# ASSERT-KTH/QuantizedSAE

Measured on AMD Instinct MI355X. Metric: activations/sec, BinarySAE 512->32768 n_bits=4 forward (dense latent + reconstruction + MSE), higher is better.
Workload: dtype f32; 1 GPU; BinarySAE(512, 32768, gamma=4.0, n_bits=4) k=65, 65536 rows per GPU per step, reference forward() signature (dense [B,32768] latent, [B,512] reconstruction, polarize loss) + recon-MSE accumulation; rows_per_gpu=65536, input_dim=512, hidden_dim=32768, n_bits=4, top_k=65, parallelism=row-sharded x1, no data-path collective, batches_in_flight=2

## Files before the change

quantizedsae_amd/_lib.py:

```python
from __future__ import annotations

import ctypes as C
from pathlib import Path
from typing import Optional

_PKG = Path(__file__).resolve().parent
import os

LIB_PATH = Path(os.environ["QSAE_HIP_LIB"]) if os.environ.get("QSAE_HIP_LIB") else _PKG / "lib" / "libqsae_hip.so"
DEBUG_LIB_PATH = _PKG / "lib" / "libqsae_hip_debug.so"
ABI_VERSION = 4

OK = 0
ERR_INVALID_ARG, ERR_UNSUPPORTED, ERR_HIP, ERR_WORKSPACE = -1, -2, -3, -4
ACT_NONE, ACT_RELU, ACT_SIGMOID = 0, 1, 2

_vp, _i, _i64, _f, _sz = C.c_void_p, C.c_int, C.c_int64, C.c_float, C.c_size_t

SIGNATURES = {
    "qsae_abi_version": (_i, []),
    "qsae_last_error": (C.c_char_p, []),
    "qsae_device_info": (_i, [C.POINTER(_i), C.c_char_p, _i]),
    "qsae_profile_sweep_events": (_i, [_vp, _vp]),
    "qsae_profile_event_create": (_i, [C.POINTER(_vp)]),
# ... 222 lines not shown
    "qsaej_threshold_grad": (_i, [_vp, _vp, _vp, _vp, _vp, _i, _i, _i, _f, _vp, _vp]),
}

JUMP_DENSE_SIGNATURES = {
    "qsaed_encode_jump_workspace_bytes": (_sz, [_i, _i, _i, _i]),
    "qsaed_encode_jump": (_i, [_vp, _i64, _vp, _i64, _vp, _vp, _i, _i, _i, _i, _f, _f, _vp, _vp, _vp, _vp, _vp, _vp, _vp, _vp, _sz,
                               _vp]),
}

BATCH_DENSE_SIGNATURES = {
    "qsaebd_encode_batch_topk_workspace_bytes": (_sz, [_i, _i, _i, _i]),
    "qsaebd_encode_batch_topk": (_i, [_vp, _i64, _vp, _i64, _vp, _i, _i, _i, _i, _i64, _vp, _f, _f, _vp, _vp, _vp, _vp, _vp, _vp,
                                      _f, _vp, _sz, _vp]),
}


class QsaeError(RuntimeError):

    def __init__(self, code: int, message: str):
        super().__init__(f"libqsae_hip error {code}: {message}")
        self.code = code


_libs = {}
_active = "product"


def _open(path: Path) -> C.CDLL:
    if not path.exists():
        raise RuntimeError(
            f"{path} is missing: build it with `python -m quantizedsae_amd.build` "
            "(hipcc --offload-arch=gfx950).  quantizedsae_amd has no CPU / eager fallback.")
    lib = C.CDLL(str(path))
    for name, (res, args) in list(SIGNATURES.items()) + list(EXT_SIGNATURES.items()) + list(CURVE_SIGNATURES.items()) \
            + list(NESTED_SIGNATURES.items()) + list(BATCH_SIGNATURES.items()) + list(NESTED_BATCH_SIGNATURES.items()) + list(MULTIK_SIGNATURES.items()) \
            + list(JUMP_SIGNATURES.items()) + list(JUMP_DENSE_SIGNATURES.items()) \
            + list(BATCH_DENSE_SIGNATURES.items()):
        fn = getattr(lib, name)
        fn.restype = res
        fn.argtypes = args
    if lib.qsae_abi_version() != ABI_VERSION:
        raise RuntimeError(f"{path.name}: ABI version mismatch; rebuild it")
    return lib


def load() -> C.CDLL:
    lib = _libs.get(_active)
    if lib is None:
        lib = _libs[_active] = _open(LIB_PATH if _active == "product" else DEBUG_LIB_PATH)
    return lib


# ... 23 lines not shown
```

quantizedsae_amd/build.py:

```python
from __future__ import annotations

import os
import shutil
import subprocess
from concurrent.futures import ThreadPoolExecutor
from pathlib import Path

PKG = Path(__file__).resolve().parent
CSRC = PKG / "csrc"
LIBDIR = PKG / "lib"
LIB = LIBDIR / "libqsae_hip.so"
DEBUG_LIB = LIBDIR / "libqsae_hip_debug.so"
OBJDIR = PKG / "lib" / "obj"

SOURCES = ["encode.hip", "topk.hip", "binary.hip", "dense_dec.hip", "encode_topk.hip", "prefilter_topk.hip", "encode_bits.hip",
           "encode_emu.hip", "misc.hip", "analysis.hip", "coactivation_bits.hip", "coactivation_partners.hip", "token_overlap.hip", "token_lists.hip", "dictionary.hip", "dictionary_neighbors.hip", "dictionary_neighbors_f32.hip", "kmeans.hip", "top_examples.hip", "evaluation.hip", "train.hip", "train_gemm.hip",
           "train_mask.hip", "optim.hip", "trainer.hip", "watch.hip", "activity.hip", "resample.hip", "auxk.hip",
           "sparsity_curve.hip", "nested.hip", "batch_topk.hip", "batch_topk_decode.hip", "nested_ragged.hip", "multi_topk.hip", "jumprelu.hip",
           "jump_dense.hip", "batch_dense.hip"]
HEADERS = sorted(p.name for p in (Path(__file__).resolve().parent / "csrc").glob("*.h"))
ARCH = "gfx950"
FLAGS = ["-O3", f"--offload-arch={ARCH}", "-ffp-contract=off", "-fPIC", "-std=c++17", "-Wall",
         "-Wno-unused-function", "-Wno-unused-variable"]

# ... 7 lines not shown

def _stale(target: Path, deps) -> bool:
    if not target.exists():
        return True
    t = target.stat().st_mtime
    return any(Path(d).stat().st_mtime > t for d in deps)


def build_native(force: bool = False, verbose: bool = False, debug: bool = False) -> Path:
    srcs = [CSRC / s for s in SOURCES if (CSRC / s).exists()]
    hdrs = [CSRC / h for h in HEADERS] + [PKG.parent / "include" / "qsae.h", PKG.parent / "include" / "qsae_ext.h",
                                        PKG.parent / "include" / "qsae_curve.h", PKG.parent / "include" / "qsae_nested.h",
                                        PKG.parent / "include" / "qsae_batch.h", PKG.parent / "include" / "qsae_nested_batch.h",
                                        PKG.parent / "include" / "qsae_multik.h", PKG.parent / "include" / "qsae_jump.h",
                                        PKG.parent / "include" / "qsae_jump_dense.h",
                                        PKG.parent / "include" / "qsae_batch_dense.h"]
    objdir = OBJDIR / "debug" if debug else OBJDIR
    lib = DEBUG_LIB if debug else LIB
    flags = FLAGS + (["-DQSAE_DEBUG_BUILD=1"] if debug else [])
    objdir.mkdir(parents=True, exist_ok=True)
    hipcc = _hipcc()
    jobs = []
    for src in srcs:
        obj = objdir / (src.stem + ".o")
        if force or _stale(obj, [src] + hdrs):
            jobs.append((src, obj))

    def compile_one(job):
        src, obj = job
        cmd = [hipcc] + flags + ["-c", str(src), "-o", str(obj)]
        if verbose:
# ... 30 lines not shown
```

quantizedsae_amd/csrc/encode_topk_internal.h:

```cpp
#pragma once

#include "gemm_mfma_f32_dma.h"
#include "decode_row.h"

namespace qsae {

int topk_rows_dispatch(float* latent, int64_t ld, int B, int H, int k, int32_t* idx, float* val, int zero_rest,
                       float* tau, uint2* cand, int* cnt, int cap, float* dense, int64_t dense_ld, hipStream_t s,
                       const float* margin = nullptr, int stride = 0);
int scatter_rows(const int32_t* idx, const float* val, int B, int k, int H, float* dense, int64_t ld, hipStream_t s);
int decode_binary_sparse_rows(const int* rows, int nrows, const int32_t* idx, const float* val, int k, int H,
                              const RowDecode& d, hipStream_t s);
int densify_rows(const int32_t* idx, const float* val, int B, int k, int H, float* dense, int64_t ld, hipStream_t s);
int gather_rows(const float* src, const int* rows, int n, int D, float* dst, hipStream_t s);
void launch_x_prep(const float* x, int B, int D, const float* meta, _Float16* xq, float* inv, float* margin, hipStream_t s,
                   int* zero_word = nullptr);

constexpr int kChunkRows = 1024;
constexpr int kTopkMaxH = 32768;
constexpr int kCandCap = 1024;
constexpr int kMaxSpecRows = kChunkRows;
constexpr int kRefMaxD = 2048;
constexpr int kRefTileStride = 36;

#ifdef QSAE_DEBUG_BUILD
// ... 157 lines not shown
```

quantizedsae_amd/csrc/misc.hip:

```cpp
#include <map>

#include "common.h"

namespace qsae {

char* last_error_buf() {
    static thread_local char buf[512] = {0};
    return buf;
}

int thread_device_ctx(ThreadDeviceCtx** out) {
    static thread_local std::map<int, ThreadDeviceCtx> table;
    int dev = -1;
    QSAE_HIP(hipGetDevice(&dev));
    auto it = table.find(dev);
    if (it == table.end()) {
        ThreadDeviceCtx c{};
        auto undo = [&c]() {
            if (c.pinned) (void)hipHostFree(c.pinned);
            if (c.ev_copied) (void)hipEventDestroy(c.ev_copied);
            if (c.ev_join) (void)hipEventDestroy(c.ev_join);
            if (c.ev_fork) (void)hipEventDestroy(c.ev_fork);
            if (c.side) (void)hipStreamDestroy(c.side);
        };
// ... 22 lines not shown
}

typedef float f32x4 __attribute__((ext_vector_type(4)));

__global__ void __launch_bounds__(256)
scatter_rows_kernel(const int32_t* __restrict__ idx, const float* __restrict__ val, long long total, int k,
                    int H, float* __restrict__ dense, int64_t ld) {
    const long long gid = static_cast<long long>(blockIdx.x) * blockDim.x + threadIdx.x;
    if (gid >= total) return;
    const long long b = gid / k;
    const int h = idx[gid];
    if (h >= 0 && h < H) dense[b * ld + h] = val[gid];
}

__global__ void __launch_bounds__(256)
sq_err_kernel(const float* __restrict__ r, const float* __restrict__ x, size_t n, double* __restrict__ sum) {
    const size_t n4 = n / 4;
    double acc = 0.0;
    const size_t stride = static_cast<size_t>(gridDim.x) * blockDim.x;
    const size_t tiles = n4 / 1024;
    double acc1 = 0.0;
    for (size_t t = blockIdx.x; t < tiles; t += gridDim.x) {
        const size_t i0 = t * 1024 + threadIdx.x;
        f32x4 a[4], b[4];
#pragma unroll
        for (int u = 0; u < 4; ++u) {
            a[u] = reinterpret_cast<const f32x4*>(r)[i0 + 256 * u];
            b[u] = reinterpret_cast<const f32x4*>(x)[i0 + 256 * u];
        }
#pragma unroll
// ... 95 lines not shown
        QSAE_HIP(hipMemset2DAsync(dense, static_cast<size_t>(ld) * sizeof(float), 0,
                                  static_cast<size_t>(H) * sizeof(float), B, s));
    }
    return scatter_rows(idx, val, B, k, H, dense, ld, s);
}

int scatter_rows(const int32_t* idx, const float* val, int B, int k, int H, float* dense, int64_t ld, hipStream_t s) {
    const long long total = static_cast<long long>(B) * k;
    if (total == 0) return QSAE_OK;
    hipLaunchKernelGGL(scatter_rows_kernel, dim3(static_cast<unsigned>((total + 255) / 256)), dim3(256), 0, s, idx,
                       val, total, k, H, dense, ld);
    QSAE_LAUNCH_CHECK();
    return QSAE_OK;
}

}

using namespace qsae;

extern "C" int qsae_kperm_rows(const float* src, int rows, int K, float* dst, qsae_stream_t stream) {
    QSAE_CHECK_ARG(rows >= 0 && K > 0, "rows >= 0 and K > 0 required");
    if (rows == 0) return QSAE_OK;
    QSAE_CHECK_ARG(src && dst && src != dst, "null or aliasing pointers");
    QSAE_CHECK_SUPPORTED(K % 8 == 0, "K must be a multiple of 8");
    QSAE_CHECK_ARG(aligned16(src) && aligned16(dst), "src and dst must be 16-byte aligned");
    const long long groups = static_cast<long long>(rows) * (K / 8);
    hipLaunchKernelGGL(kperm_rows_kernel, dim3(static_cast<unsigned>((groups + 255) / 256)), dim3(256), 0,
                       as_stream(stream), src, groups, dst);
    QSAE_LAUNCH_CHECK();
    return QSAE_OK;
// ... 129 lines not shown
```

quantizedsae_amd/csrc/prefilter_topk.hip:

```cpp
#ifdef QSAE_DEBUG_BUILD
#define QSAE_DEFINE_SHARED_TUNABLES 1
#endif
#include "encode_topk_internal.h"
#include "sweep_xstat_f16.h"
#include "refine_row.h"
#include "refine_sliced.h"

namespace qsae {

constexpr int kFillCoWaves = 1024;
constexpr int kFillCoPace = 3;

QSAE_TUNABLE_PTR g_xstat_stamps = nullptr;
QSAE_TUNABLE g_fuse_xprep = 0;
QSAE_TUNABLE g_inkernel_pilot = 1;
QSAE_TUNABLE g_inkernel_rank = 0;
QSAE_TUNABLE g_pilot_tile = 0;
QSAE_TUNABLE g_fill_in_sweep = 1;
QSAE_TUNABLE g_fill_co = 1;
QSAE_TUNABLE g_xstat_ablate = 0;
QSAE_TUNABLE g_x_parts = 0;
QSAE_TUNABLE g_pref_tile = 2;

struct PrefLayout {
// ... 228 lines not shown
    return fits == 1;
}

static int launch_fill_co(ThreadDeviceCtx* ctx, float* dense, int64_t dense_ld, int B, int H, hipStream_t s) {
    QSAE_HIP(hipStreamWaitEvent(ctx->side, ctx->ev_fork, 0));
    hipLaunchKernelGGL(co_delay_kernel, dim3(1), dim3(64), 0, ctx->side, 2000);
    QSAE_LAUNCH_CHECK();
    hipLaunchKernelGGL(fill_zero_co_kernel, dim3(g_fill_co > 1 ? g_fill_co % 10000 : kFillCoWaves), dim3(64), 0, ctx->side,
                       dense, static_cast<long long>(dense_ld), B, H / 256, g_fill_co > 1 ? g_fill_co / 10000 : kFillCoPace);
    QSAE_LAUNCH_CHECK();
    QSAE_HIP(hipEventRecord(ctx->ev_join, ctx->side));
    QSAE_HIP(hipStreamWaitEvent(s, ctx->ev_join, 0));
    return QSAE_OK;
}

static bool prefilter_shape_ok(int B, int D, int H, int k) {
    return use_fused(B, D, H, k) && D % 64 == 0 && D <= kRefMaxD && (H - pilot_width(H)) > 0;
}

static int inkernel_rank(int k) {
    const double target = 5.0 * k > 200.0 ? 5.0 * k : 200.0;
    int r = static_cast<int>(32.0 * (1.0 - exp(-target / 512.0)) + 0.5);
    return r < 6 ? 6 : (r > 24 ? 24 : r);
}

struct PrefCall {
    const float* x; const float* W; const float* bias; const _Float16* Wq; const float* meta;
    int B, D, H, k;
    int32_t* idx; float* val;
    char* ws; qsae_stream_t stream;
    float* dense; int64_t dense_ld;
    const RowDecode* dec;
};
struct PrefPlan {
    FusedLayout L; PrefLayout PL;
    int P;
    bool xstat, inkernel, fill_co, fill_in_sweep;
    int Hs, hoff, parts, cap_part;
    float* filled;
};
static PrefPlan pref_plan(const PrefCall& c) {
    PrefPlan p;
    p.L = fused_layout(c.B, c.D, c.H, c.k);
    p.PL = pref_layout(c.B, c.D, p.L.total);
    p.P = pilot_width(c.H);
    p.xstat = g_pref_tile == 2 && xstat_supported(c.D, c.H - p.P, p.P) && c.H % 4 == 0;
    p.inkernel = p.xstat && g_inkernel_pilot && p.P % kXsHT == 0 && c.H % kXsHT == 0 && xstat_supported(c.D, c.H, 0);
    p.Hs = p.inkernel ? c.H : c.H - p.P;
    p.hoff = p.inkernel ? 0 : p.P;
    p.parts = p.xstat ? (g_x_parts > 0 ? g_x_parts : xstat_parts(c.B, p.Hs, kCandCap)) : 1;
    p.cap_part = kCandCap / p.parts;
    p.fill_co = p.xstat && c.dense && g_fill_co && c.D == 512 && c.H % 256 == 0 && c.dense_ld % 4 == 0 && g_xstat_ablate == 0 &&
                co_fill_fits();
    p.fill_in_sweep = !p.fill_co && p.xstat && c.dense && g_fill_in_sweep && c.H % 256 == 0 && c.dense_ld % 4 == 0;
    p.filled = (p.fill_in_sweep || p.fill_co) ? c.dense : nullptr;
    return p;
}

static int prefilter_submit(const PrefCall& c) {
    hipStream_t s = as_stream(c.stream);
    const SweepProfile prof = take_sweep_profile();
    const PrefPlan pl = pref_plan(c);
    const FusedLayout& L = pl.L;
    const PrefLayout& PL = pl.PL;
    const int B = c.B, D = c.D, H = c.H, k = c.k, P = pl.P;
    char* ws = c.ws;
    float* pilot = reinterpret_cast<float*>(ws + L.pilot);
    float* tau = reinterpret_cast<float*>(ws + L.tau);
    int* cnt = reinterpret_cast<int*>(ws + L.cnt);
    uint2* cand = reinterpret_cast<uint2*>(ws + L.cand);
    int* flags = reinterpret_cast<int*>(ws + L.flags);
    _Float16* xq = reinterpret_cast<_Float16*>(ws + PL.xq);
    float* inv = reinterpret_cast<float*>(ws + PL.inv);
    float* margin = reinterpret_cast<float*>(ws + PL.margin);
    int* cnt_parts = reinterpret_cast<int*>(ws + PL.cnt_parts);
    const bool xstat = pl.xstat, inkernel = pl.inkernel, fill_co = pl.fill_co, fill_in_sweep = pl.fill_in_sweep;
    float* fused_fill = xstat ? nullptr : c.dense;
    const int Hs = pl.Hs, hoff = pl.hoff, parts = pl.parts, cap_part = pl.cap_part;
    const int xs_iters = xstat ? (Hs / kXsHT) / parts + (inkernel ? P / kXsHT : 0) : 0;
    const int fill_cw = xs_iters > 0 ? (32 * (H / 256) / parts + xs_iters - 1) / xs_iters : 0;
    ThreadDeviceCtx* ctx = nullptr;
    if (fill_co) {
        const int rc0 = thread_device_ctx(&ctx);
        if (rc0 != QSAE_OK) return rc0;
    }
    const bool fuse_prep = inkernel && g_fuse_xprep;
    if (!fuse_prep && (g_x_phase & 1)) {
        launch_x_prep(c.x, B, D, c.meta, xq, inv, margin, s, flags);
        QSAE_LAUNCH_CHECK();
    } else {
        QSAE_HIP(hipMemsetAsync(flags, 0, sizeof(int), s));
    }
    const int Kw = D / 2;
    const float* xq_w = reinterpret_cast<const float*>(xq);
    const float* wq_w = reinterpret_cast<const float*>(c.Wq);
    int rc = QSAE_OK;
    if (!inkernel) {
        if (g_pilot_tile == 0 && P % 256 == 0) {
// ... 11 lines not shown
    if (!inkernel) rc = topk_rows_dispatch(pilot, P, B, P, j, nullptr, nullptr, 0, tau, cand, cnt, cap_part, fused_fill, c.dense_ld, s,
                                margin, kCandCap);
    if (rc != QSAE_OK) return rc;
    if (g_x_phase & 1) {
        using EpiS = EpiFilter<256, 128, 4, 2, true>;
        typename EpiS::Args es{c.bias ? c.bias + P : nullptr, tau, cand, cnt, kCandCap, P, fused_fill, c.dense_ld, inv, margin};
        if (prof.begin) QSAE_HIP(hipEventRecord(prof.begin, s));
        if (xstat) {
            XsArgs xa{};
            xa.xq = xq;  xa.wq = c.Wq + static_cast<size_t>(hoff) * D;  xa.bias = c.bias ? c.bias + hoff : nullptr;  xa.tau = tau;
            xa.margin = margin;  xa.inv = inv;  xa.cand = cand;  xa.cnt = cnt;  xa.B = B;  xa.Hs = Hs;  xa.cap = kCandCap;
            xa.hidden_offset = hoff;  xa.rot_mul = g_xstat_rot;  xa.stamps = g_xstat_stamps;  xa.H = H;  xa.fill_cw = fill_cw;
            xa.dense = fill_in_sweep ? c.dense : nullptr;  xa.dense_ld = c.dense_ld;  xa.pilot_stages = inkernel ? P / kXsHT : 0;
            xa.pilot_rank = g_inkernel_rank > 0 ? g_inkernel_rank : inkernel_rank(k);  xa.tau_out = tau;  xa.meta = c.meta;
            xa.x32 = fuse_prep ? c.x : nullptr;  xa.inv_out = inv;  xa.margin_out = margin;  xa.parts = parts;  xa.cnt_parts = cnt_parts;
            if (fill_co) QSAE_HIP(hipEventRecord(ctx->ev_fork, s));
            rc = launch_xstat(D, xa, s, (g_xstat_ablate == 0 && D == 512 && !fill_in_sweep) ? 9 : g_xstat_ablate);
            if (fill_co && rc == QSAE_OK) rc = launch_fill_co(ctx, c.dense, c.dense_ld, B, H, s);
        } else if (g_pref_tile != 1) {
            using EpiW = EpiFilter<256, 256, 4, 2, true>;
            typename EpiW::Args ew{es.bias, es.tau, es.cand, es.cnt, es.cap, es.hidden_offset, es.dense, es.dense_ld, es.inv,
                                   es.margin};
            rc = launch_gemm_dma<EpiW, 256, 256, true, 2>(wq_w + static_cast<size_t>(P) * Kw, H - P, xq_w, B, Kw, ew, s);
        } else {
            rc = launch_gemm_dma<EpiS, 256, 128, true>(wq_w + static_cast<size_t>(P) * Kw, H - P, xq_w, B, Kw, es, s);
        }
        if (prof.end) QSAE_HIP(hipEventRecord(prof.end, s));
        if (rc != QSAE_OK) return rc;
        if (xstat && g_xstat_ablate != 0) return QSAE_OK;
    }
    if (g_x_phase & 2) {
        const RowDecode rd = c.dec ? *c.dec : RowDecode{nullptr, 0, 0, 0, 0, 0.f, nullptr, nullptr, nullptr};
        if (refine_sliced_wanted(B, D, H, k))
// ... 218 lines not shown
        call.dec = &dec;
    } else if (table) {
        if (!recon) return fail(QSAE_ERR_INVALID_ARG, "%s: invalid argument: table given without recon", who);
        if (!(aligned16(table) && aligned16(recon)))
            return fail(QSAE_ERR_INVALID_ARG, "%s: invalid argument: table and recon must be 16-byte aligned", who);
        dec = RowDecode{nullptr, 0, 0, 0, D, step, dec_bias, recon, table};
        call.dec = &dec;
    }
    return QSAE_OK;
}

enum class PrefMode { blocking, submit, finish };
static int prefilter_entry(const char* who, PrefMode mode, bool need_dict, const float* x, const float* W, const float* bias,
                           const void* Wq, const float* meta, int B, int D, int H, int k, const uint8_t* packed, int n_bits, float step,
                           const float* table, const float* dec_bias, int32_t* idx, float* val, float* dense, int64_t dense_ld,
                           float* recon, void* workspace, size_t workspace_bytes, int n, int* out, qsae_stream_t stream) {
    if (!(B >= 0 && D > 0 && H > 0)) return fail(QSAE_ERR_INVALID_ARG, "%s: invalid argument: B >= 0, D > 0, H > 0 required", who);
    if (mode == PrefMode::submit && !out)
        return fail(QSAE_ERR_INVALID_ARG, "%s: invalid argument: flagged_host must point to a host int", who);
    if (out && (mode == PrefMode::blocking || B == 0)) *out = 0;
    if (B == 0) return QSAE_OK;
    if (need_dict && !((packed || table) && recon)) return fail(QSAE_ERR_INVALID_ARG, "%s: invalid argument: null pointer", who);
    PrefCall call;
    RowDecode dec;
    int rc = prefilter_call(who, x, W, bias, Wq, meta, B, D, H, k, packed, n_bits, step, dec_bias, idx, val, dense, dense_ld, recon,
                            workspace, workspace_bytes, stream, call, dec, table);
    if (rc != QSAE_OK) return rc;
    if (mode == PrefMode::blocking) return run_prefilter(call, n, out);
    if (mode == PrefMode::finish) return prefilter_finish(call, 0, n);
    rc = prefilter_submit(call);
    if (rc != QSAE_OK) return rc;
    QSAE_HIP(hipMemcpyAsync(out, call.ws + pref_plan(call).L.flags, sizeof(int), hipMemcpyDeviceToHost, as_stream(stream)));
    return QSAE_OK;
}

extern "C" int qsae_encode_topk_prefilter(const float* x, const float* W, const float* bias, const void* Wq,
                                          const float* meta, int B, int D, int H, int k, int32_t* idx, float* val,
                                          float* dense, int64_t dense_ld, void* workspace, size_t workspace_bytes,
                                          int spec_rows, int* flagged_rows, qsae_stream_t stream) {
    return prefilter_entry(__func__, PrefMode::blocking, false, x, W, bias, Wq, meta, B, D, H, k, nullptr, 0, 0.f, nullptr, nullptr, idx,
                           val, dense, dense_ld, nullptr, workspace, workspace_bytes, spec_rows, flagged_rows, stream);
}
// ... 38 lines not shown
extern "C" int qsae_prefilter_submit_table(const float* x, const float* W, const float* bias, const void* Wq, const float* meta,
                                           int B, int D, int H, int k, const float* table, float scale, const float* dec_bias,
                                           int32_t* idx, float* val, float* dense, int64_t dense_ld, float* recon,
                                           void* workspace, size_t workspace_bytes, int* flagged_host, qsae_stream_t stream) {
    return prefilter_entry(__func__, PrefMode::submit, true, x, W, bias, Wq, meta, B, D, H, k, nullptr, 0, scale, table, dec_bias, idx,
                           val, dense, dense_ld, recon, workspace, workspace_bytes, 0, flagged_host, stream);
}

extern "C" int qsae_prefilter_finish_table(const float* x, const float* W, const float* bias, const void* Wq, const float* meta,
                                           int B, int D, int H, int k, const float* table, float scale, const float* dec_bias,
                                           int32_t* idx, float* val, float* dense, int64_t dense_ld, float* recon,
                                           void* workspace, size_t workspace_bytes, int flagged, qsae_stream_t stream) {
    return prefilter_entry(__func__, PrefMode::finish, true, x, W, bias, Wq, meta, B, D, H, k, nullptr, 0, scale, table, dec_bias, idx,
                           val, dense, dense_ld, recon, workspace, workspace_bytes, flagged, nullptr, stream);
}
```

quantizedsae_amd/ops.py:

```python
from __future__ import annotations

import collections
import ctypes as C
import functools
import weakref
from typing import Callable, NamedTuple, Optional, Tuple

import torch

from . import _lib
from ._lib import ACT_NONE, ACT_RELU, ACT_SIGMOID, check


def _stream() -> C.c_void_p:
    return C.c_void_p(torch.cuda.current_stream().cuda_stream)


def _on_tensor_device(fn):
    @functools.wraps(fn)
    def wrapper(*args, **kwargs):
        for a in args:
            if isinstance(a, torch.Tensor):
                if a.is_cuda and a.device.index != torch.cuda.current_device():
                    with torch.cuda.device(a.device):
# ... 232 lines not shown
    slot = (owner, slot)
    _claim_slot(x.device, slot)
    cargs, keep, z = _encode_bits_fp16_cargs(x, W, b, Wq, meta, B, D, H, _workspace(x.device, need, slot, "pending"))
    lib = _lib.load()
    return _submit(getattr(lib, _BITS_FP16[kind][2]), getattr(lib, _BITS_FP16[kind][3]), cargs, keep, z, x.device, slot)


@_on_tensor_device
def topk_rows(latent: torch.Tensor, k: int, zero_rest: bool) -> Tuple[torch.Tensor, torch.Tensor]:
    _dev(latent, "latent", torch.float32)
    if latent.dim() != 2 or latent.stride(1) != 1:
        raise ValueError("latent must be a 2-D tensor with unit inner stride")
    B, H = latent.shape
    idx = torch.empty((B, k), dtype=torch.int32, device=latent.device)
    val = torch.empty((B, k), dtype=torch.float32, device=latent.device)
    check(_lib.load().qsae_topk_rows(_p(latent), latent.stride(0) if B else H, B, H, k, _p(idx), _p(val),
                                     1 if zero_rest else 0, _stream()))
    return idx, val


_workspaces = collections.OrderedDict()
WORKSPACE_CACHE_PER_DEVICE = 6
_busy_slots = {}


def _workspace(device: torch.device, nbytes: int, slot: int = 0, kind: str = "call") -> torch.Tensor:
    dev = device.index if device.index is not None else torch.cuda.current_device()
    key = (dev, torch.cuda.current_stream(device).cuda_stream, kind, slot)
    ws = _workspaces.get(key)
    if ws is None or ws.numel() < nbytes:
        ws = torch.empty((max(nbytes, 1),), dtype=torch.uint8, device=device)
        _workspaces[key] = ws
    _workspaces.move_to_end(key)
    mine = [k for k in _workspaces if k[0] == dev]
    for k in mine[:max(0, len(mine) - WORKSPACE_CACHE_PER_DEVICE)]:
        ref = _busy_slots.get((k[0], k[1], k[3])) if k[2] == "pending" else None
        if ref is not None and ref() is not None:
            continue
        del _workspaces[k]
    return ws


def release_workspaces() -> None:
    _workspaces.clear()


def encode_topk_supported(B: int, D: int, H: int, k: int) -> bool:
    return int(_lib.load().qsae_encode_topk_workspace_bytes(B, D, H, k)) > 0


def _encode_topk_workspace(lib, B: int, D: int, H: int, k: int) -> int:
    need = int(lib.qsae_encode_topk_workspace_bytes(B, D, H, k))
    if need == 0 and B > 0:
        raise ValueError(f"encode_topk: shape B={B}, D={D}, H={H}, k={k} is outside what the kernels run (fused form: "
                         "B >= 2048, 8192 <= H <= 65536; otherwise H <= 32768; H % 4 == 0, D % 4 == 0, k <= 256)")
    return need


@_on_tensor_device
# ... 54 lines not shown
    B, D = x.shape
    H = W.shape[0]
    b = _f32c(bias, "bias") if bias is not None else None
    lib = _lib.load()
    need = int(lib.qsae_encode_topk_prefilter_workspace_bytes(B, D, H, k))
    if need == 0:
        raise ValueError("shape not supported by the fp16 prefilter")
    ws = _workspace(x.device, need)
    idx = torch.empty((B, k), dtype=torch.int32, device=x.device)
    val = torch.empty((B, k), dtype=torch.float32, device=x.device)
    if dense_out is not None:
        _dev(dense_out, "dense_out", torch.float32)
        if dense_out.dim() != 2 or dense_out.shape[0] != B or dense_out.shape[1] < H or dense_out.stride(1) != 1:
            raise ValueError("dense_out must be a [B, >=H] fp32 tensor with unit column stride")
        dense, ld = dense_out, dense_out.stride(0)
    else:
        dense = torch.empty((B, H), dtype=torch.float32, device=x.device) if want_dense else None
        ld = H
    flagged = C.c_int(0)
    kernel_timer.arm_sweep()
    check(lib.qsae_encode_topk_prefilter(_p(x), _p(W), _p(b), _p(Wq), _p(meta), B, D, H, k, _p(idx), _p(val),
                                         _p(dense), ld, _p(ws), ws.numel(), int(spec_rows), C.byref(flagged), _stream()))
    if info is not None:
        info["flagged_rows"] = int(flagged.value)
    return idx, val, (dense[:, :H] if dense_out is not None else dense)


def _decode_prefilter_args(x, W, bias, Wq, meta, k, decoder, dec_bias, want_dense, slot, kind):
    x, W = _f32c(x, "x"), _f32c(W, "W")
    B, D = x.shape
# ... 2 lines not shown
    db = _f32c(dec_bias, "dec_bias") if dec_bias is not None else None
    if decoder[0] == "packed":
        dict_t = _dev(decoder[1], "packed", torch.uint8)
        dargs = (_p(dict_t), int(decoder[2]), float(decoder[3]))
    else:
        dict_t = _f32c(decoder[1], "table")
        if tuple(dict_t.shape) != (H, D):
            raise ValueError(f"table is {tuple(dict_t.shape)}, expected [{H}, {D}]")
        dargs = (_p(dict_t), float(decoder[2]))
    need = int(_lib.load().qsae_encode_topk_prefilter_workspace_bytes(B, D, H, k))
    if need == 0:
        raise ValueError("shape not supported by the fp16 prefilter")
    ws = _workspace(x.device, need, slot, kind)
    idx = torch.empty((B, k), dtype=torch.int32, device=x.device)
    val = torch.empty((B, k), dtype=torch.float32, device=x.device)
    dense = torch.empty((B, H), dtype=torch.float32, device=x.device) if want_dense else None
    recon = torch.empty((B, D), dtype=torch.float32, device=x.device)
    cargs = (_p(x), _p(W), _p(b), _p(Wq), _p(meta), B, D, H, k) + dargs + (_p(db), _p(idx), _p(val), _p(dense), H, _p(recon),
                                                                          _p(ws), ws.numel())
    keep = (x, W, b, Wq, meta, dict_t, db, ws)
    return cargs, keep, (idx, val, dense, recon)


_PREFILTER_FORWARD = {"packed": "qsae_binary_forward_prefilter", "table": "qsae_table_forward_prefilter"}
_PREFILTER_SUBMIT = {"packed": ("qsae_prefilter_submit", "qsae_prefilter_finish"),
                     "table": ("qsae_prefilter_submit_table", "qsae_prefilter_finish_table")}


@_on_tensor_device
def _forward_prefilter(x, W, bias, Wq, meta, k, decoder, dec_bias, want_dense, spec_rows, info):
    cargs, keep, outs = _decode_prefilter_args(x, W, bias, Wq, meta, k, decoder, dec_bias, want_dense, 0, "call")
    flagged = C.c_int(0)
    kernel_timer.arm_sweep()
    check(getattr(_lib.load(), _PREFILTER_FORWARD[decoder[0]])(*cargs, int(spec_rows), C.byref(flagged), _stream()))
    if info is not None:
        info["flagged_rows"] = int(flagged.value)
    return outs


def binary_forward_prefilter(x: torch.Tensor, W: torch.Tensor, bias: Optional[torch.Tensor], Wq: torch.Tensor,
                             meta: torch.Tensor, k: int, packed: torch.Tensor, n_bits: int, step: float,
                             dec_bias: Optional[torch.Tensor], want_dense: bool = True, spec_rows: int = 0,
                             info: Optional[dict] = None):
    return _forward_prefilter(x, W, bias, Wq, meta, k, ("packed", packed, n_bits, step), dec_bias, want_dense, spec_rows, info)


def table_forward_prefilter(x: torch.Tensor, W: torch.Tensor, bias: Optional[torch.Tensor], Wq: torch.Tensor,
                            meta: torch.Tensor, k: int, table: torch.Tensor, scale: float,
                            dec_bias: Optional[torch.Tensor], want_dense: bool = True, spec_rows: int = 0,
                            info: Optional[dict] = None):
    return _forward_prefilter(x, W, bias, Wq, meta, k, ("table", table, scale), dec_bias, want_dense, spec_rows, info)


class PendingForward:

    def __init__(self, finish_fn, cargs, keep, outs, word, event, device, stream, slot_key):
        self._finish_fn, self._cargs, self._keep, self._outs = finish_fn, cargs, keep, outs
        self._word, self._event, self._device, self._stream, self._slot_key = word, event, device, stream, slot_key
        self.flagged_rows = None
        _busy_slots[slot_key] = weakref.ref(self)

    def _release(self):
        ref = _busy_slots.get(self._slot_key)
        if ref is not None and ref() in (self, None):
            del _busy_slots[self._slot_key]
        self._cargs = self._keep = None

    def finish(self):
        if self._cargs is None:
            return self._outs
        self._event.synchronize()
        self.flagged_rows = int(self._word.item())
        try:
            with torch.cuda.device(self._device), torch.cuda.stream(self._stream):
                check(self._finish_fn(*self._cargs, self.flagged_rows, _stream()))
        finally:
            self._release()
        return self._outs

    def __del__(self):
        try:
            if self._cargs is not None:
                self._event.synchronize()
                self._release()
        except Exception:
            pass


def _submit(submit_fn, finish_fn, cargs, keep, outs, device, slot):
    stream = torch.cuda.current_stream(device)
    slot_key = (device.index if device.index is not None else torch.cuda.current_device(), stream.cuda_stream, slot)
    word = torch.zeros((1,), dtype=torch.int32).pin_memory()
    kernel_timer.arm_sweep()
    check(submit_fn(*cargs, C.c_void_p(word.data_ptr()), _stream()))
    ev = torch.cuda.Event()
    ev.record(stream)
    return PendingForward(finish_fn, cargs, keep, outs, word, ev, device, stream, slot_key)


def _claim_slot(device, slot):
    key = (device.index if device.index is not None else torch.cuda.current_device(),
           torch.cuda.current_stream(device).cuda_stream, slot)
    ref = _busy_slots.get(key)
    if ref is not None and ref() is None:
        del _busy_slots[key]
        ref = None
    if ref is not None:
        raise RuntimeError(f"submit: slot {slot[-1] if isinstance(slot, tuple) else slot} of this stream still holds a batch whose finish() / result() has not been "
                           "called; batches in flight together need different slot numbers")


@_on_tensor_device
def _forward_prefilter_submit(x, W, bias, Wq, meta, k, decoder, dec_bias, want_dense, slot, owner) -> PendingForward:
    slot = (owner, slot)
    _claim_slot(x.device, slot)
    cargs, keep, outs = _decode_prefilter_args(x, W, bias, Wq, meta, k, decoder, dec_bias, want_dense, slot, "pending")
    lib = _lib.load()
    submit_fn, finish_fn = (getattr(lib, name) for name in _PREFILTER_SUBMIT[decoder[0]])
    return _submit(submit_fn, finish_fn, cargs, keep, outs, x.device, slot)


def binary_forward_prefilter_submit(x: torch.Tensor, W: torch.Tensor, bias: Optional[torch.Tensor], Wq: torch.Tensor,
                                    meta: torch.Tensor, k: int, packed: torch.Tensor, n_bits: int, step: float,
                                    dec_bias: Optional[torch.Tensor], want_dense: bool = True,
                                    slot: int = 0, owner: int = 0) -> PendingForward:
    return _forward_prefilter_submit(x, W, bias, Wq, meta, k, ("packed", packed, n_bits, step), dec_bias, want_dense, slot,
                                     owner)


def table_forward_prefilter_submit(x: torch.Tensor, W: torch.Tensor, bias: Optional[torch.Tensor], Wq: torch.Tensor,
                                   meta: torch.Tensor, k: int, table: torch.Tensor, scale: float,
                                   dec_bias: Optional[torch.Tensor], want_dense: bool = True,
                                   slot: int = 0, owner: int = 0) -> PendingForward:
    return _forward_prefilter_submit(x, W, bias, Wq, meta, k, ("table", table, scale), dec_bias, want_dense, slot, owner)


@_on_tensor_device
def densify(idx: torch.Tensor, val: torch.Tensor, H: int, out: Optional[torch.Tensor] = None) -> torch.Tensor:
    _dev(idx, "idx", torch.int32)
    _dev(val, "val", torch.float32)
    B, k = idx.shape
    if out is None:
        out = torch.empty((B, H), dtype=torch.float32, device=idx.device)
    check(_lib.load().qsae_densify(_p(idx.contiguous()), _p(val.contiguous()), B, k, H, _p(out),
                                   out.stride(0) if B else H, _stream()))
    return out


def binary_row_bytes(D: int, n_bits: int) -> int:
    r = int(_lib.load().qsae_binary_row_bytes(D, n_bits))
    if r < 0:
        check(r)
    return r


@_on_tensor_device
def pack_binary(logits: torch.Tensor, D: int, n_bits: int, want_polarize: bool = True, want_soft_gap: bool = False):
    logits = _f32c(logits, "logits")
# ... 1068 lines not shown
def _levels_grad(g_levels: Optional[torch.Tensor], n_bits: int, B: int, D: int):
    if g_levels is None:
        return None
    g = _f32c(g_levels, "g_levels")
    if tuple(g.shape) != (n_bits, B, D):
        raise ValueError(f"g_levels is {tuple(g.shape)}, expected [{n_bits}, {B}, {D}]")
    return g


@_on_tensor_device
def train_matryoshka_dpre(pre: torch.Tensor, g_levels: Optional[torch.Tensor], g_groups: Optional[torch.Tensor],
                          sign_rows: torch.Tensor, scale: torch.Tensor, sizes) -> torch.Tensor:
    _dev(pre, "pre", torch.float32)
    if pre.dim() != 2 or not pre.is_contiguous():
        raise ValueError("train_matryoshka_dpre: pre must be a contiguous [B, H] tensor (it is updated in place)")
    B, H = pre.shape
    sign_rows, scale = _f32c(sign_rows, "sign_rows"), _f32c(scale, "scale")
    D = sign_rows.shape[1]
    _check_matryoshka_shape(D)
    n_bits = len(sizes)
    if sign_rows.shape[0] != H or scale.numel() != H or sum(sizes) != H or B < 1:
        raise ValueError("train_matryoshka_dpre: inconsistent shapes")
    G = _levels_grad(g_levels, n_bits, B, D)
    gg = _f32c(g_groups.reshape(-1), "g_groups") if g_groups is not None else None
    if gg is not None and gg.numel() != n_bits:
        raise ValueError(f"g_groups has {gg.numel()} elements, expected {n_bits}")
    keep, sp = _sizes_arg(sizes, n_bits)
    check(_lib.load().qsae_train_matryoshka_dpre(_p(G), _p(gg), _p(sign_rows), _p(scale), B, D, H, n_bits, sp, _p(pre), H,
                                                 _stream()))
    return pre
# ... 168 lines not shown
            or pre.numel() >= 2 ** 31:
        raise ValueError(f"blatent_binarize: pre must be a contiguous [B, H] tensor with H a multiple of 32, B >= 1 and "
                         f"B * H below 2^31, got {tuple(pre.shape)}")
    B, H = pre.shape
    latent = torch.empty_like(pre) if want_latent else None
    zbits = torch.empty((B, H // 32), dtype=torch.int32, device=pre.device)
    check(_lib.load().qsae_blatent_binarize(_p(pre), B, H, float(cutoff), _p(latent), _p(zbits), _stream()))
    return latent, zbits


@_on_tensor_device
def train_blatent_dpre(pre: torch.Tensor, g_recon: torch.Tensor, w_dec: torch.Tensor) -> torch.Tensor:
    _dev(pre, "pre", torch.float32)
    if pre.dim() != 2 or not pre.is_contiguous():
        raise ValueError("train_blatent_dpre: pre must be a contiguous [B, H] tensor (it is updated in place)")
    B, H = pre.shape
    G, w_dec = _f32c(g_recon, "g_recon"), _f32c(w_dec, "w_dec")
    D = w_dec.shape[0]
    if not train_blatent_supported(D, H) or B < 1 or B * H >= 2 ** 31:
        raise ValueError(f"train_blatent_dpre: {_BLATENT_LIMITS} (got B = {B}, D = {D}, H = {H})")
    if tuple(w_dec.shape) != (D, H) or tuple(G.shape) != (B, D):
        raise ValueError("train_blatent_dpre: inconsistent shapes")
    check(_lib.load().qsae_train_blatent_dpre(_p(G), _p(w_dec), B, D, H, _p(pre), _stream()))
    return pre


@_on_tensor_device
def train_blatent_dweight(g_recon: torch.Tensor, zbits: torch.Tensor, H: int) -> torch.Tensor:
    _dev(zbits, "zbits", torch.int32)
    G = _f32c(g_recon, "g_recon")
# ... 1236 lines not shown
```

Measured before the change: 17.79 million activations/s.

## Recycle released dense latent buffers and erase only stale top-k entries

Adds a per-device, per-stream pool of dense [B,H] latent buffers that the caller no longer holds. When a forward call can reuse one, it clears only the previous call's k non-zero entries per row, using a new erase kernel on the main or side stream, instead of zero-filling the whole dense latent. This is meant to remove the full-matrix zero fill, which is a large memory write for a 32768-wide latent. In exchange it adds version and held-reference bookkeeping in Python, new recycled ABI entry points, and risks returning stale data if something writes to the buffer outside the tracked paths.

Result: faster. 19.52 million activations/s (median of 6 runs) (+9.7%).

```diff
diff --git a/include/qsae_recycle.h b/include/qsae_recycle.h
--- /dev/null
+++ b/include/qsae_recycle.h
@@ -0,0 +1,41 @@
+#ifndef QSAE_RECYCLE_H
+#define QSAE_RECYCLE_H
+
+#include "qsae.h"
+
+#ifdef __cplusplus
+extern "C" {
+#endif
+
+#define QSAER_MAX_STALE_K 1024
+
+int qsaer_binary_forward_prefilter(const float* x, const float* W, const float* bias, const void* Wq,
+                                   const float* meta, int B, int D, int H, int k, const uint8_t* packed, int n_bits,
+                                   float step, const float* dec_bias, int32_t* idx, float* val, float* dense,
+                                   int64_t dense_ld, float* recon, void* workspace, size_t workspace_bytes,
+                                   int spec_rows, int* flagged_rows, qsae_stream_t stream, const int32_t* stale_idx,
+                                   int stale_k);
+
+int qsaer_table_forward_prefilter(const float* x, const float* W, const float* bias, const void* Wq, const float* meta,
+                                  int B, int D, int H, int k, const float* table, float scale, const float* dec_bias,
+                                  int32_t* idx, float* val, float* dense, int64_t dense_ld, float* recon, void* workspace,
+                                  size_t workspace_bytes, int spec_rows, int* flagged_rows, qsae_stream_t stream,
+                                  const int32_t* stale_idx, int stale_k);
+
+int qsaer_prefilter_submit(const float* x, const float* W, const float* bias, const void* Wq, const float* meta,
+                           int B, int D, int H, int k, const uint8_t* packed, int n_bits, float step,
+                           const float* dec_bias, int32_t* idx, float* val, float* dense, int64_t dense_ld,
+                           float* recon, void* workspace, size_t workspace_bytes, int* flagged_host,
+                           qsae_stream_t stream, const int32_t* stale_idx, int stale_k);
+
+int qsaer_prefilter_submit_table(const float* x, const float* W, const float* bias, const void* Wq, const float* meta,
+                                 int B, int D, int H, int k, const float* table, float scale, const float* dec_bias,
+                                 int32_t* idx, float* val, float* dense, int64_t dense_ld, float* recon, void* workspace,
+                                 size_t workspace_bytes, int* flagged_host, qsae_stream_t stream,
+                                 const int32_t* stale_idx, int stale_k);
+
+#ifdef __cplusplus
+}
+#endif
+
+#endif
diff --git a/quantizedsae_amd/_lib.py b/quantizedsae_amd/_lib.py
--- a/quantizedsae_amd/_lib.py
+++ b/quantizedsae_amd/_lib.py
@@ -260,6 +260,12 @@
                                       _f, _vp, _sz, _vp]),
 }
 
+RECYCLE_SIGNATURES = {
+    "qsaer_" + name[len("qsae_"):]: (SIGNATURES[name][0], SIGNATURES[name][1] + [_vp, _i])
+    for name in ("qsae_binary_forward_prefilter", "qsae_table_forward_prefilter", "qsae_prefilter_submit",
+                 "qsae_prefilter_submit_table")
+}
+
 
 class QsaeError(RuntimeError):
 
@@ -281,7 +287,7 @@
     for name, (res, args) in list(SIGNATURES.items()) + list(EXT_SIGNATURES.items()) + list(CURVE_SIGNATURES.items()) \
             + list(NESTED_SIGNATURES.items()) + list(BATCH_SIGNATURES.items()) + list(NESTED_BATCH_SIGNATURES.items()) + list(MULTIK_SIGNATURES.items()) \
             + list(JUMP_SIGNATURES.items()) + list(JUMP_DENSE_SIGNATURES.items()) \
-            + list(BATCH_DENSE_SIGNATURES.items()):
+            + list(BATCH_DENSE_SIGNATURES.items()) + list(RECYCLE_SIGNATURES.items()):
         fn = getattr(lib, name)
         fn.restype = res
         fn.argtypes = args
diff --git a/quantizedsae_amd/build.py b/quantizedsae_amd/build.py
--- a/quantizedsae_amd/build.py
+++ b/quantizedsae_amd/build.py
@@ -45,7 +45,8 @@
                                         PKG.parent / "include" / "qsae_batch.h", PKG.parent / "include" / "qsae_nested_batch.h",
                                         PKG.parent / "include" / "qsae_multik.h", PKG.parent / "include" / "qsae_jump.h",
                                         PKG.parent / "include" / "qsae_jump_dense.h",
-                                        PKG.parent / "include" / "qsae_batch_dense.h"]
+                                        PKG.parent / "include" / "qsae_batch_dense.h",
+                                        PKG.parent / "include" / "qsae_recycle.h"]
     objdir = OBJDIR / "debug" if debug else OBJDIR
     lib = DEBUG_LIB if debug else LIB
     flags = FLAGS + (["-DQSAE_DEBUG_BUILD=1"] if debug else [])
diff --git a/quantizedsae_amd/csrc/encode_topk_internal.h b/quantizedsae_amd/csrc/encode_topk_internal.h
--- a/quantizedsae_amd/csrc/encode_topk_internal.h
+++ b/quantizedsae_amd/csrc/encode_topk_internal.h
@@ -9,6 +9,7 @@
                        float* tau, uint2* cand, int* cnt, int cap, float* dense, int64_t dense_ld, hipStream_t s,
                        const float* margin = nullptr, int stride = 0);
 int scatter_rows(const int32_t* idx, const float* val, int B, int k, int H, float* dense, int64_t ld, hipStream_t s);
+int erase_rows(const int32_t* idx, int B, int k, int H, float* dense, int64_t ld, hipStream_t s);
 int decode_binary_sparse_rows(const int* rows, int nrows, const int32_t* idx, const float* val, int k, int H,
                               const RowDecode& d, hipStream_t s);
 int densify_rows(const int32_t* idx, const float* val, int B, int k, int H, float* dense, int64_t ld, hipStream_t s);
diff --git a/quantizedsae_amd/csrc/misc.hip b/quantizedsae_amd/csrc/misc.hip
--- a/quantizedsae_amd/csrc/misc.hip
+++ b/quantizedsae_amd/csrc/misc.hip
@@ -60,6 +60,15 @@
 }
 
 __global__ void __launch_bounds__(256)
+erase_rows_kernel(const int32_t* __restrict__ idx, long long total, int k, int H, float* __restrict__ dense, int64_t ld) {
+    const long long gid = static_cast<long long>(blockIdx.x) * blockDim.x + threadIdx.x;
+    if (gid >= total) return;
+    const long long b = gid / k;
+    const uint32_t h = static_cast<uint32_t>(idx[gid]);
+    if (h < static_cast<uint32_t>(H)) dense[b * ld + h] = 0.0f;
+}
+
+__global__ void __launch_bounds__(256)
 sq_err_kernel(const float* __restrict__ r, const float* __restrict__ x, size_t n, double* __restrict__ sum) {
     const size_t n4 = n / 4;
     double acc = 0.0;
@@ -185,6 +194,15 @@
     return QSAE_OK;
 }
 
+int erase_rows(const int32_t* idx, int B, int k, int H, float* dense, int64_t ld, hipStream_t s) {
+    const long long total = static_cast<long long>(B) * k;
+    if (total == 0) return QSAE_OK;
+    hipLaunchKernelGGL(erase_rows_kernel, dim3(static_cast<unsigned>((total + 255) / 256)), dim3(256), 0, s, idx, total, k, H,
+                       dense, ld);
+    QSAE_LAUNCH_CHECK();
+    return QSAE_OK;
+}
+
 }
 
 using namespace qsae;
diff --git a/quantizedsae_amd/csrc/prefilter_topk.hip b/quantizedsae_amd/csrc/prefilter_topk.hip
--- a/quantizedsae_amd/csrc/prefilter_topk.hip
+++ b/quantizedsae_amd/csrc/prefilter_topk.hip
@@ -5,6 +5,7 @@
 #include "sweep_xstat_f16.h"
 #include "refine_row.h"
 #include "refine_sliced.h"
+#include "../../include/qsae_recycle.h"
 
 namespace qsae {
 
@@ -266,6 +267,18 @@
     return QSAE_OK;
 }
 
+static int launch_erase_co(ThreadDeviceCtx* ctx, const int32_t* stale_idx, int stale_k, float* dense, int64_t dense_ld, int B, int H,
+                           hipStream_t s) {
+    QSAE_HIP(hipStreamWaitEvent(ctx->side, ctx->ev_fork, 0));
+    hipLaunchKernelGGL(co_delay_kernel, dim3(1), dim3(64), 0, ctx->side, 2000);
+    QSAE_LAUNCH_CHECK();
+    const int rc = erase_rows(stale_idx, B, stale_k, H, dense, dense_ld, ctx->side);
+    if (rc != QSAE_OK) return rc;
+    QSAE_HIP(hipEventRecord(ctx->ev_join, ctx->side));
+    QSAE_HIP(hipStreamWaitEvent(s, ctx->ev_join, 0));
+    return QSAE_OK;
+}
+
 static bool prefilter_shape_ok(int B, int D, int H, int k) {
     return use_fused(B, D, H, k) && D % 64 == 0 && D <= kRefMaxD && (H - pilot_width(H)) > 0;
 }
@@ -283,6 +296,7 @@
     char* ws; qsae_stream_t stream;
     float* dense; int64_t dense_ld;
     const RowDecode* dec;
+    const int32_t* stale_idx; int stale_k;
 };
 struct PrefPlan {
     FusedLayout L; PrefLayout PL;
@@ -290,6 +304,7 @@
     bool xstat, inkernel, fill_co, fill_in_sweep;
     int Hs, hoff, parts, cap_part;
     float* filled;
+    bool recycled;
 };
 static PrefPlan pref_plan(const PrefCall& c) {
     PrefPlan p;
@@ -306,6 +321,7 @@
                 co_fill_fits();
     p.fill_in_sweep = !p.fill_co && p.xstat && c.dense && g_fill_in_sweep && c.H % 256 == 0 && c.dense_ld % 4 == 0;
     p.filled = (p.fill_in_sweep || p.fill_co) ? c.dense : nullptr;
+    p.recycled = c.stale_idx != nullptr && p.filled != nullptr;
     return p;
 }
 
@@ -326,14 +342,19 @@
     float* inv = reinterpret_cast<float*>(ws + PL.inv);
     float* margin = reinterpret_cast<float*>(ws + PL.margin);
     int* cnt_parts = reinterpret_cast<int*>(ws + PL.cnt_parts);
-    const bool xstat = pl.xstat, inkernel = pl.inkernel, fill_co = pl.fill_co, fill_in_sweep = pl.fill_in_sweep;
+    const bool xstat = pl.xstat, inkernel = pl.inkernel, fill_co = pl.fill_co && !pl.recycled,
+               fill_in_sweep = pl.fill_in_sweep && !pl.recycled, erase_co = pl.recycled && pl.fill_co && (g_x_phase & 1);
     float* fused_fill = xstat ? nullptr : c.dense;
     const int Hs = pl.Hs, hoff = pl.hoff, parts = pl.parts, cap_part = pl.cap_part;
     const int xs_iters = xstat ? (Hs / kXsHT) / parts + (inkernel ? P / kXsHT : 0) : 0;
     const int fill_cw = xs_iters > 0 ? (32 * (H / 256) / parts + xs_iters - 1) / xs_iters : 0;
     ThreadDeviceCtx* ctx = nullptr;
-    if (fill_co) {
+    if (fill_co || erase_co) {
         const int rc0 = thread_device_ctx(&ctx);
+        if (rc0 != QSAE_OK) return rc0;
+    }
+    if (pl.recycled && !erase_co) {
+        const int rc0 = erase_rows(c.stale_idx, B, c.stale_k, H, c.dense, c.dense_ld, s);
         if (rc0 != QSAE_OK) return rc0;
     }
     const bool fuse_prep = inkernel && g_fuse_xprep;
@@ -375,9 +396,10 @@
             xa.dense = fill_in_sweep ? c.dense : nullptr;  xa.dense_ld = c.dense_ld;  xa.pilot_stages = inkernel ? P / kXsHT : 0;
             xa.pilot_rank = g_inkernel_rank > 0 ? g_inkernel_rank : inkernel_rank(k);  xa.tau_out = tau;  xa.meta = c.meta;
             xa.x32 = fuse_prep ? c.x : nullptr;  xa.inv_out = inv;  xa.margin_out = margin;  xa.parts = parts;  xa.cnt_parts = cnt_parts;
-            if (fill_co) QSAE_HIP(hipEventRecord(ctx->ev_fork, s));
+            if (fill_co || erase_co) QSAE_HIP(hipEventRecord(ctx->ev_fork, s));
             rc = launch_xstat(D, xa, s, (g_xstat_ablate == 0 && D == 512 && !fill_in_sweep) ? 9 : g_xstat_ablate);
             if (fill_co && rc == QSAE_OK) rc = launch_fill_co(ctx, c.dense, c.dense_ld, B, H, s);
+            if (erase_co && rc == QSAE_OK) rc = launch_erase_co(ctx, c.stale_idx, c.stale_k, c.dense, c.dense_ld, B, H, s);
         } else if (g_pref_tile != 1) {
             using EpiW = EpiFilter<256, 256, 4, 2, true>;
             typename EpiW::Args ew{es.bias, es.tau, es.cand, es.cnt, es.cap, es.hidden_offset, es.dense, es.dense_ld, es.inv,
@@ -626,7 +648,8 @@
 static int prefilter_entry(const char* who, PrefMode mode, bool need_dict, const float* x, const float* W, const float* bias,
                            const void* Wq, const float* meta, int B, int D, int H, int k, const uint8_t* packed, int n_bits, float step,
                            const float* table, const float* dec_bias, int32_t* idx, float* val, float* dense, int64_t dense_ld,
-                           float* recon, void* workspace, size_t workspace_bytes, int n, int* out, qsae_stream_t stream) {
+                           float* recon, void* workspace, size_t workspace_bytes, int n, int* out, qsae_stream_t stream,
+                           const int32_t* stale_idx = nullptr, int stale_k = 0) {
     if (!(B >= 0 && D > 0 && H > 0)) return fail(QSAE_ERR_INVALID_ARG, "%s: invalid argument: B >= 0, D > 0, H > 0 required", who);
     if (mode == PrefMode::submit && !out)
         return fail(QSAE_ERR_INVALID_ARG, "%s: invalid argument: flagged_host must point to a host int", who);
@@ -638,6 +661,13 @@
     int rc = prefilter_call(who, x, W, bias, Wq, meta, B, D, H, k, packed, n_bits, step, dec_bias, idx, val, dense, dense_ld, recon,
                             workspace, workspace_bytes, stream, call, dec, table);
     if (rc != QSAE_OK) return rc;
+    if (stale_idx) {
+        if (!(stale_k >= 1 && stale_k <= QSAER_MAX_STALE_K && (reinterpret_cast<uintptr_t>(stale_idx) & 3u) == 0))
+            return fail(QSAE_ERR_INVALID_ARG, "%s: invalid argument: 1 <= stale_k <= %d and a 4-byte aligned stale_idx required", who,
+                        QSAER_MAX_STALE_K);
+        call.stale_idx = stale_idx;
+        call.stale_k = stale_k;
+    }
     if (mode == PrefMode::blocking) return run_prefilter(call, n, out);
     if (mode == PrefMode::finish) return prefilter_finish(call, 0, n);
     rc = prefilter_submit(call);
@@ -706,3 +736,42 @@
     return prefilter_entry(__func__, PrefMode::finish, true, x, W, bias, Wq, meta, B, D, H, k, nullptr, 0, scale, table, dec_bias, idx,
                            val, dense, dense_ld, recon, workspace, workspace_bytes, flagged, nullptr, stream);
 }
+
+extern "C" int qsaer_binary_forward_prefilter(const float* x, const float* W, const float* bias, const void* Wq,
+                                              const float* meta, int B, int D, int H, int k, const uint8_t* packed,
+                                              int n_bits, float step, const float* dec_bias, int32_t* idx, float* val,
+                                              float* dense, int64_t dense_ld, float* recon, void* workspace,
+                                              size_t workspace_bytes, int spec_rows, int* flagged_rows,
+                                              qsae_stream_t stream, const int32_t* stale_idx, int stale_k) {
+    return prefilter_entry(__func__, PrefMode::blocking, true, x, W, bias, Wq, meta, B, D, H, k, packed, n_bits, step, nullptr, dec_bias,
+                           idx, val, dense, dense_ld, recon, workspace, workspace_bytes, spec_rows, flagged_rows, stream, stale_idx,
+                           stale_k);
+}
+
+extern "C" int qsaer_table_forward_prefilter(const float* x, const float* W, const float* bias, const void* Wq,
+                                             const float* meta, int B, int D, int H, int k, const float* table, float scale,
+                                             const float* dec_bias, int32_t* idx, float* val, float* dense, int64_t dense_ld,
+                                             float* recon, void* workspace, size_t workspace_bytes, int spec_rows,
+                                             int* flagged_rows, qsae_stream_t stream, const int32_t* stale_idx, int stale_k) {
+    return prefilter_entry(__func__, PrefMode::blocking, true, x, W, bias, Wq, meta, B, D, H, k, nullptr, 0, scale, table, dec_bias, idx,
+                           val, dense, dense_ld, recon, workspace, workspace_bytes, spec_rows, flagged_rows, stream, stale_idx,
+                           stale_k);
+}
+
+extern "C" int qsaer_prefilter_submit(const float* x, const float* W, const float* bias, const void* Wq, const float* meta,
+                                      int B, int D, int H, int k, const uint8_t* packed, int n_bits, float step,
+                                      const float* dec_bias, int32_t* idx, float* val, float* dense, int64_t dense_ld,
+                                      float* recon, void* workspace, size_t workspace_bytes, int* flagged_host,
+                                      qsae_stream_t stream, const int32_t* stale_idx, int stale_k) {
+    return prefilter_entry(__func__, PrefMode::submit, false, x, W, bias, Wq, meta, B, D, H, k, packed, n_bits, step, nullptr, dec_bias,
+                           idx, val, dense, dense_ld, recon, workspace, workspace_bytes, 0, flagged_host, stream, stale_idx, stale_k);
+}
+
+extern "C" int qsaer_prefilter_submit_table(const float* x, const float* W, const float* bias, const void* Wq, const float* meta,
+                                            int B, int D, int H, int k, const float* table, float scale, const float* dec_bias,
+                                            int32_t* idx, float* val, float* dense, int64_t dense_ld, float* recon,
+                                            void* workspace, size_t workspace_bytes, int* flagged_host, qsae_stream_t stream,
+                                            const int32_t* stale_idx, int stale_k) {
+    return prefilter_entry(__func__, PrefMode::submit, true, x, W, bias, Wq, meta, B, D, H, k, nullptr, 0, scale, table, dec_bias, idx,
+                           val, dense, dense_ld, recon, workspace, workspace_bytes, 0, flagged_host, stream, stale_idx, stale_k);
+}
diff --git a/quantizedsae_amd/ops.py b/quantizedsae_amd/ops.py
--- a/quantizedsae_amd/ops.py
+++ b/quantizedsae_amd/ops.py
@@ -3,6 +3,8 @@
 import collections
 import ctypes as C
 import functools
+import sys
+import threading
 import weakref
 from typing import Callable, NamedTuple, Optional, Tuple
 
@@ -270,6 +272,8 @@
     B, H = latent.shape
     idx = torch.empty((B, k), dtype=torch.int32, device=latent.device)
     val = torch.empty((B, k), dtype=torch.float32, device=latent.device)
+    if zero_rest:
+        _latent_pool_forget(latent)
     check(_lib.load().qsae_topk_rows(_p(latent), latent.stride(0) if B else H, B, H, k, _p(idx), _p(val),
                                      1 if zero_rest else 0, _stream()))
     return idx, val
@@ -299,6 +303,69 @@
 
 def release_workspaces() -> None:
     _workspaces.clear()
+    with _latent_pool_lock:
+        del _latent_pool[:]
+
+
+LATENT_RECYCLE = True
+LATENT_POOL_PER_DEVICE = 4
+_LatentRecord = collections.namedtuple("_LatentRecord", "key dense idx dense_version idx_version")
+_latent_pool = []
+_latent_pool_lock = threading.Lock()
+latent_pool_stats = {"hits": 0, "misses": 0}
+_latent_holder_baseline = None
+
+
+def _latent_holders(rec):
+    dense = rec.dense
+    storage = dense.untyped_storage()
+    return (sys.getrefcount(dense), dense._use_count(), torch._C._storage_Use_Count(storage._cdata), sys.getrefcount(storage))
+
+
+def _latent_unheld(rec) -> bool:
+    global _latent_holder_baseline
+    if _latent_holder_baseline is None:
+        _latent_holder_baseline = _latent_holders(_LatentRecord(None, torch.empty((1, 1)), None, 0, 0))
+    return _latent_holders(rec) == _latent_holder_baseline
+
+
+def _latent_pool_take(key):
+    with _latent_pool_lock:
+        edited = [r for r in _latent_pool if r.dense._version != r.dense_version or r.idx._version != r.idx_version]
+        if edited:
+            _latent_pool[:] = [r for r in _latent_pool if not any(r is e for e in edited)]
+        for i, rec in enumerate(_latent_pool):
+            if rec.key == key and _latent_unheld(rec):
+                del _latent_pool[i]
+                latent_pool_stats["hits"] += 1
+                return rec.dense, rec.idx
+        latent_pool_stats["misses"] += 1
+    return None
+
+
+def _latent_pool_register(key, dense, idx) -> None:
+    try:
+        rec = _LatentRecord(key, dense, idx, dense._version, idx._version)
+    except RuntimeError:
+        return
+    with _latent_pool_lock:
+        _latent_pool.append(rec)
+        mine = [r for r in _latent_pool if r.key[0] == key[0]]
+        drop = mine[:max(0, len(mine) - LATENT_POOL_PER_DEVICE)]
+        if drop:
+            _latent_pool[:] = [r for r in _latent_pool if not any(r is d for d in drop)]
+
+
+def _latent_pool_forget(t: torch.Tensor) -> None:
+    if not _latent_pool:
+        return
+    ptr = t.untyped_storage().data_ptr()
+    with _latent_pool_lock:
+        _latent_pool[:] = [r for r in _latent_pool if r.dense.untyped_storage().data_ptr() != ptr]
+
+
+def _recycled(name: str, tail) -> str:
+    return "qsaer_" + name[len("qsae_"):] if tail else name
 
 
 def encode_topk_supported(B: int, D: int, H: int, k: int) -> bool:
@@ -383,6 +450,7 @@
         if dense_out.dim() != 2 or dense_out.shape[0] != B or dense_out.shape[1] < H or dense_out.stride(1) != 1:
             raise ValueError("dense_out must be a [B, >=H] fp32 tensor with unit column stride")
         dense, ld = dense_out, dense_out.stride(0)
+        _latent_pool_forget(dense_out)
     else:
         dense = torch.empty((B, H), dtype=torch.float32, device=x.device) if want_dense else None
         ld = H
@@ -415,12 +483,18 @@
     ws = _workspace(x.device, need, slot, kind)
     idx = torch.empty((B, k), dtype=torch.int32, device=x.device)
     val = torch.empty((B, k), dtype=torch.float32, device=x.device)
-    dense = torch.empty((B, H), dtype=torch.float32, device=x.device) if want_dense else None
+    dense = stale = pool_key = None
+    if want_dense and LATENT_RECYCLE:
+        dev = x.device.index if x.device.index is not None else torch.cuda.current_device()
+        pool_key = (dev, torch.cuda.current_stream(x.device).cuda_stream, B, H, k)
+        dense, stale = _latent_pool_take(pool_key) or (None, None)
+    if want_dense and dense is None:
+        dense = torch.empty((B, H), dtype=torch.float32, device=x.device)
     recon = torch.empty((B, D), dtype=torch.float32, device=x.device)
     cargs = (_p(x), _p(W), _p(b), _p(Wq), _p(meta), B, D, H, k) + dargs + (_p(db), _p(idx), _p(val), _p(dense), H, _p(recon),
                                                                           _p(ws), ws.numel())
-    keep = (x, W, b, Wq, meta, dict_t, db, ws)
-    return cargs, keep, (idx, val, dense, recon)
+    keep = (x, W, b, Wq, meta, dict_t, db, ws, stale)
+    return cargs, keep, (idx, val, dense, recon), pool_key, ((_p(stale), k) if stale is not None else ())
 
 
 _PREFILTER_FORWARD = {"packed": "qsae_binary_forward_prefilter", "table": "qsae_table_forward_prefilter"}
@@ -430,10 +504,13 @@
 
 @_on_tensor_device
 def _forward_prefilter(x, W, bias, Wq, meta, k, decoder, dec_bias, want_dense, spec_rows, info):
-    cargs, keep, outs = _decode_prefilter_args(x, W, bias, Wq, meta, k, decoder, dec_bias, want_dense, 0, "call")
+    cargs, keep, outs, pool_key, tail = _decode_prefilter_args(x, W, bias, Wq, meta, k, decoder, dec_bias, want_dense, 0, "call")
     flagged = C.c_int(0)
     kernel_timer.arm_sweep()
-    check(getattr(_lib.load(), _PREFILTER_FORWARD[decoder[0]])(*cargs, int(spec_rows), C.byref(flagged), _stream()))
+    fn = getattr(_lib.load(), _recycled(_PREFILTER_FORWARD[decoder[0]], tail))
+    check(fn(*cargs, int(spec_rows), C.byref(flagged), _stream(), *tail))
+    if pool_key is not None:
+        _latent_pool_register(pool_key, outs[2], outs[0])
     if info is not None:
         info["flagged_rows"] = int(flagged.value)
     return outs
@@ -455,9 +532,10 @@
 
 class PendingForward:
 
-    def __init__(self, finish_fn, cargs, keep, outs, word, event, device, stream, slot_key):
+    def __init__(self, finish_fn, cargs, keep, outs, word, event, device, stream, slot_key, latent_record=None):
         self._finish_fn, self._cargs, self._keep, self._outs = finish_fn, cargs, keep, outs
         self._word, self._event, self._device, self._stream, self._slot_key = word, event, device, stream, slot_key
+        self._latent_record = latent_record
         self.flagged_rows = None
         _busy_slots[slot_key] = weakref.ref(self)
 
@@ -465,7 +543,7 @@
         ref = _busy_slots.get(self._slot_key)
         if ref is not None and ref() in (self, None):
             del _busy_slots[self._slot_key]
-        self._cargs = self._keep = None
+        self._cargs = self._keep = self._latent_record = None
 
     def finish(self):
         if self._cargs is None:
@@ -475,6 +553,8 @@
         try:
             with torch.cuda.device(self._device), torch.cuda.stream(self._stream):
                 check(self._finish_fn(*self._cargs, self.flagged_rows, _stream()))
+            if self._latent_record is not None:
+                _latent_pool_register(*self._latent_record)
         finally:
             self._release()
         return self._outs
@@ -488,15 +568,15 @@
             pass
 
 
-def _submit(submit_fn, finish_fn, cargs, keep, outs, device, slot):
+def _submit(submit_fn, finish_fn, cargs, keep, outs, device, slot, tail=(), latent_record=None):
     stream = torch.cuda.current_stream(device)
     slot_key = (device.index if device.index is not None else torch.cuda.current_device(), stream.cuda_stream, slot)
     word = torch.zeros((1,), dtype=torch.int32).pin_memory()
     kernel_timer.arm_sweep()
-    check(submit_fn(*cargs, C.c_void_p(word.data_ptr()), _stream()))
+    check(submit_fn(*cargs, C.c_void_p(word.data_ptr()), _stream(), *tail))
     ev = torch.cuda.Event()
     ev.record(stream)
-    return PendingForward(finish_fn, cargs, keep, outs, word, ev, device, stream, slot_key)
+    return PendingForward(finish_fn, cargs, keep, outs, word, ev, device, stream, slot_key, latent_record)
 
 
 def _claim_slot(device, slot):
@@ -515,10 +595,12 @@
 def _forward_prefilter_submit(x, W, bias, Wq, meta, k, decoder, dec_bias, want_dense, slot, owner) -> PendingForward:
     slot = (owner, slot)
     _claim_slot(x.device, slot)
-    cargs, keep, outs = _decode_prefilter_args(x, W, bias, Wq, meta, k, decoder, dec_bias, want_dense, slot, "pending")
-    lib = _lib.load()
-    submit_fn, finish_fn = (getattr(lib, name) for name in _PREFILTER_SUBMIT[decoder[0]])
-    return _submit(submit_fn, finish_fn, cargs, keep, outs, x.device, slot)
+    cargs, keep, outs, pool_key, tail = _decode_prefilter_args(x, W, bias, Wq, meta, k, decoder, dec_bias, want_dense, slot,
+                                                               "pending")
+    lib = _lib.load()
+    submit_name, finish_name = _PREFILTER_SUBMIT[decoder[0]]
+    return _submit(getattr(lib, _recycled(submit_name, tail)), getattr(lib, finish_name), cargs, keep, outs, x.device, slot,
+                   tail=tail, latent_record=(pool_key, outs[2], outs[0]) if pool_key is not None else None)
 
 
 def binary_forward_prefilter_submit(x: torch.Tensor, W: torch.Tensor, bias: Optional[torch.Tensor], Wq: torch.Tensor,
@@ -543,6 +625,8 @@
     B, k = idx.shape
     if out is None:
         out = torch.empty((B, H), dtype=torch.float32, device=idx.device)
+    else:
+        _latent_pool_forget(out)
     check(_lib.load().qsae_densify(_p(idx.contiguous()), _p(val.contiguous()), B, k, H, _p(out),
                                    out.stride(0) if B else H, _stream()))
     return out
@@ -1641,6 +1725,7 @@
     _dev(pre, "pre", torch.float32)
     if pre.dim() != 2 or not pre.is_contiguous():
         raise ValueError("train_matryoshka_dpre: pre must be a contiguous [B, H] tensor (it is updated in place)")
+    _latent_pool_forget(pre)
     B, H = pre.shape
     sign_rows, scale = _f32c(sign_rows, "sign_rows"), _f32c(scale, "scale")
     D = sign_rows.shape[1]
@@ -1839,6 +1924,7 @@
     _dev(pre, "pre", torch.float32)
     if pre.dim() != 2 or not pre.is_contiguous():
         raise ValueError("train_blatent_dpre: pre must be a contiguous [B, H] tensor (it is updated in place)")
+    _latent_pool_forget(pre)
     B, H = pre.shape
     G, w_dec = _f32c(g_recon, "g_recon"), _f32c(w_dec, "w_dec")
     D = w_dec.shape[0]
```
